# cvjena/mvlm

Hardware: NVIDIA B200
Metric: scans/sec (higher is better)
Workload: dtype bf16

## Files before the change

mvlm_b200/csrc/hourglass.cu:

```cuda
#include "hourglass.cuh"

#include <math.h>
#include <stdlib.h>

#include <algorithm>

namespace mvlm {

namespace {

__global__ void fold_bn_kernel(const float* w, const float* b, const float* m, const float* v, float eps, int n,
                               float* scale, float* shift) {
  const int i = blockIdx.x * blockDim.x + threadIdx.x;
  if (i >= n) return;
  const float s = w[i] / sqrtf(v[i] + eps);
  scale[i] = s;
  shift[i] = b[i] - m[i] * s;
}

__global__ void pack_conv_weight_kernel(const float* __restrict__ w, int cout, int cin, int kh, int kw,
                                        int cout_pad, int cin_pad, __nv_bfloat16* __restrict__ out) {
  const long long total = 1ll * cout_pad * kw * kh * cin_pad;
  for (long long i = blockIdx.x * 1ll * blockDim.x + threadIdx.x; i < total;
       i += 1ll * gridDim.x * blockDim.x) {
// ... 60 lines not shown
}

int pack_conv_weight(const float* w_oihw, int cout, int cin, int kh, int kw, int cout_pad, int cin_pad,
                     __nv_bfloat16* out, cudaStream_t stream) {
  const long long total = 1ll * cout_pad * kw * kh * cin_pad;
  const int block = 256;
  const int grid = static_cast<int>((total + block - 1) / block > 4096 ? 4096 : (total + block - 1) / block);
  pack_conv_weight_kernel<<<grid, block, 0, stream>>>(w_oihw, cout, cin, kh, kw, cout_pad, cin_pad, out);
  MVLM_CHECK_CUDA(cudaGetLastError());
  return MVLM_OK;
}

HourglassNet::~HourglassNet() {
  for (auto& g : graphs_) cudaGraphExecDestroy(g.second);
  for (void* p : owned_) cudaFree(p);
}

static uint8_t* const kFakeBase = reinterpret_cast<uint8_t*>(static_cast<uintptr_t>(1) << 44);

void* HourglassNet::ws_alloc(size_t bytes) {
  const size_t aligned = (bytes + 1023) & ~static_cast<size_t>(1023);
  if (layout_pass_) {
    Buf b;
    b.bytes = aligned;
    b.fake_off = fake_off_;
    bufs_.push_back(b);
    fake_off_ += aligned;
    return kFakeBase + b.fake_off;
  }
  if (ws_ == nullptr || next_buf_ >= bufs_.size()) return nullptr;
  return ws_ + bufs_[next_buf_++].offset;
}

void HourglassNet::note_use(const void* p) {
  if (!layout_pass_ || p == nullptr) return;
  const uint8_t* q = static_cast<const uint8_t*>(p);
  if (q < kFakeBase || q >= kFakeBase + fake_off_) return;
  const size_t off = static_cast<size_t>(q - kFakeBase);
  size_t lo = 0, hi = bufs_.size();
  while (hi - lo > 1) {
    const size_t mid = (lo + hi) / 2;
    if (bufs_[mid].fake_off <= off) lo = mid; else hi = mid;
  }
  Buf& b = bufs_[lo];
  const int op = static_cast<int>(ops_.size());
  if (b.first < 0) b.first = op;
  b.last = std::max(b.last, op);
}

void HourglassNet::note_conv(const void* in, const ConvEpilogue& e) {
  note_use(in); note_use(e.out_pre); note_use(e.res1); note_use(e.res2); note_use(e.res_up); note_use(e.out_raw);
  note_use(e.out_post); note_use(e.argmax_keys); note_use(e.out_aux1); note_use(e.out_aux2);
}

void HourglassNet::assign_offsets() {
  const int n_ops = static_cast<int>(ops_.size());
  for (Buf& b : bufs_) {
    if (b.first < 0) { b.first = 0; b.last = n_ops; }
    if (b.pinned || !reuse_) { b.first = 0; b.last = n_ops; }
  }
  std::vector<size_t> order(bufs_.size());
  for (size_t i = 0; i < order.size(); ++i) order[i] = i;
  std::stable_sort(order.begin(), order.end(), [&](size_t a, size_t b) { return bufs_[a].first < bufs_[b].first; });
  struct Block { size_t off, bytes; };
  std::vector<Block> free_list;
  std::vector<size_t> live;
  size_t top = 0;
  auto release = [&](size_t id) {
    Block nb = {bufs_[id].offset, bufs_[id].bytes};
    size_t k = 0;
    while (k < free_list.size() && free_list[k].off < nb.off) ++k;
    free_list.insert(free_list.begin() + k, nb);
    for (size_t j = 0; j + 1 < free_list.size();) {
      if (free_list[j].off + free_list[j].bytes == free_list[j + 1].off) {
        free_list[j].bytes += free_list[j + 1].bytes;
        free_list.erase(free_list.begin() + j + 1);
      } else {
        ++j;
      }
    }
    if (!free_list.empty() && free_list.back().off + free_list.back().bytes == top) {
      top = free_list.back().off;
      free_list.pop_back();
    }
  };
  for (size_t id : order) {
    Buf& b = bufs_[id];
    for (size_t j = 0; j < live.size();) {
      if (bufs_[live[j]].last < b.first) {
// ... 95 lines not shown
}

int HourglassNet::stem_weight(const __nv_bfloat16** out) {
  void* buf;
  const float* src;
  const int rc = param("conv1.weight", 64ll * cin_ * 9, sizeof(__nv_bfloat16) * 64 * 9 * 16, &buf, &src);
  *out = static_cast<__nv_bfloat16*>(buf);
  if (rc || layout_pass_) return rc;
  pack_stem_weight_kernel<<<36, 256, 0, build_stream_>>>(src, 64, cin_, 64, static_cast<__nv_bfloat16*>(buf));
  MVLM_CHECK_CUDA(cudaGetLastError());
  return MVLM_OK;
}

int HourglassNet::phase_weight(int a, int b, const __nv_bfloat16** out) {
  void* buf;
  const float* src;
  const int rc = param("conv11.weight", 9ll * L_ * L_, sizeof(__nv_bfloat16) * Lp_ * 4 * Lp_, &buf, &src);
  *out = static_cast<__nv_bfloat16*>(buf);
  if (rc || layout_pass_) return rc;
  pack_phase_weight_kernel<<<64, 256, 0, build_stream_>>>(src, L_, L_, a, b, Lp_, Lp_, static_cast<__nv_bfloat16*>(buf));
  MVLM_CHECK_CUDA(cudaGetLastError());
  return MVLM_OK;
}

int HourglassNet::emit_conv(const char* tag, T in, int cin, const __nv_bfloat16* w, int cout_pad, int n_tile, int kh,
                            int kw, int y_off0, int x_off0, const ConvEpilogue& e, double flops, bool is_head) {
  flops_ += flops;
  note_conv(in.p, e);
  NetOp op;
  op.kind = NetOp::CONV;
  op.tag = tag;
  op.is_head = is_head;
  op.h = in.h; op.w = in.w;
  if (!layout_pass_) {
    ConvShape s;
    s.in = in.p; s.n = V_; s.h = in.h; s.w = in.w; s.cin = cin; s.in_cs = in.c;
    s.wpacked = w; s.cout_pad = cout_pad; s.n_tile = n_tile; s.kh = kh; s.kw = kw;
    s.y_off0 = y_off0; s.x_off0 = x_off0;
    const int rc = conv_plan(s, e, &op.conv);
    if (rc) return rc;
  }
  ops_.push_back(op);
  return MVLM_OK;
}

int HourglassNet::rb(const std::string& p, T x, T a_in, T ar, int cin, int cout, const char* post_bn, T* post_act,
                     T* y_out, T* pool_raw, const T* up_low, const RbAux* aux) {
  const int h = a_in.h, w = a_in.w;
  T y = alloc(h, w, cout);
  T skip = x;
  int rc;
  if (cin != cout) {
    ConvEpilogue e;
    e.out_raw = y.p; e.raw_cs = cout; e.raw_co = 0;
    const __nv_bfloat16* wr;
    if ((rc = packed(p + ".resample.2.weight", cout, cin, 1, cout, cin, &wr)) ||
        (rc = emit_conv("rb.resample", ar, cin, wr, cout, cout < 128 ? cout : 128, 1, 1, 0, 0, e,
                        2.0 * cout * cin * ar.h * ar.w)))
      return rc;
    skip = y;
  }
  const float *ps = nullptr, *pt = nullptr;
  if (post_bn) {
    rc = bn(post_bn, cout, &ps, &pt);
    if (rc) return rc;
    *post_act = pool_raw ? alloc(h / 2, w / 2, cout) : alloc(h, w, cout);
  }
  if (pool_raw) *pool_raw = alloc(h / 2, w / 2, cout);
  const float *as = nullptr, *at = nullptr;
  if (aux) {
    rc = bn(aux->bn, cout, &as, &at);
    if (rc) return rc;
    *aux->out1 = aux->mode == 2 ? alloc(h / 2, w / 2, cout) : alloc(h, w, cout);
// ... 27 lines not shown
    }
    if (aux) {
      e.aux_mode = aux->mode;
      e.aux_scale = layout_pass_ ? nullptr : as + offs[i];
      e.aux_shift = layout_pass_ ? nullptr : at + offs[i];
      e.out_aux1 = aux->out1->p; e.aux1_cs = cout; e.aux1_co = offs[i];
      if (aux->mode == 2) { e.out_aux2 = aux->out2->p; e.aux2_cs = cout; e.aux2_co = offs[i]; }
    }
    const int nt = widths[i] < 128 ? widths[i] : 128;
    const __nv_bfloat16* wc;
    if ((rc = packed(p + names[i] + ".weight", widths[i], cins[i], 3, widths[i], cins[i], &wc)) ||
        (rc = emit_conv("rb.conv", ins[i], cins[i], wc, widths[i], nt, 3, 3, -1, -1, e,
                        2.0 * widths[i] * cins[i] * 9 * h * w)))
      return rc;
  }
  *y_out = y;
  return MVLM_OK;
}

int HourglassNet::emit_pool(T in, T out_raw, const char* bn_name, T out_act) {
  note_use(in.p); note_use(out_raw.p); note_use(out_act.p);
  NetOp op;
  op.kind = NetOp::POOL;
  op.in0 = in.p; op.out_raw = out_raw.p; op.out_act = out_act.p;
  op.h = in.h; op.w = in.w; op.c = in.c;
  if (bn_name) {
    int rc = bn(bn_name, in.c, &op.scale, &op.shift);
    if (rc) return rc;
  }
  ops_.push_back(op);
  return MVLM_OK;
}

int HourglassNet::hourglass(const std::string& p, T x, T a_x, T* out, const T* in_pooled, const T* in_pooled_act) {
  const int F = 256;
  int rc;
  T none;
  T lows[5], a_lows[5];
  T cur = x;
  const int low_blocks[5] = {2, 4, 6, 8, 10};
  const int skip_blocks[4] = {3, 5, 7, 9};
  T pooled, a;
  if (in_pooled) {
    pooled = *in_pooled;
    a = *in_pooled_act;
  }
  for (int lvl = 0; lvl < 5; ++lvl) {
    const std::string lb = p + ".rb" + std::to_string(low_blocks[lvl]);
    if (!(fuse_elt_ && (lvl > 0 || in_pooled))) {
      pooled = alloc(cur.h / 2, cur.w / 2, F);
      a = alloc(cur.h / 2, cur.w / 2, F);
      rc = emit_pool(cur, pooled, (lb + ".bn1").c_str(), a);
      if (rc) return rc;
    }
    const int nxt = lvl < 4 ? skip_blocks[lvl] : 11;
    const std::string post = p + ".rb" + std::to_string(nxt) + ".bn1";
    T next_pooled, next_a;
    const std::string next_bn = lvl < 4 ? p + ".rb" + std::to_string(low_blocks[lvl + 1]) + ".bn1" : "";
    RbAux aux = {2, next_bn.c_str(), &next_pooled, &next_a};
    rc = rb(lb, pooled, a, none, F, F, post.c_str(), &a_lows[lvl], &lows[lvl], nullptr, nullptr,
            (fuse_elt_ && lvl < 4) ? &aux : nullptr);
    if (rc) return rc;
    cur = lows[lvl];
    pooled = next_pooled;
    a = next_a;
  }
  T low2, a2, low3;
  rc = rb(p + ".rb11", cur, a_lows[4], none, F, F, (p + ".rb12.bn1").c_str(), &a2, &low2);
  if (rc) return rc;
  rc = rb(p + ".rb12", low2, a2, none, F, F, nullptr, nullptr, &low3);
  if (rc) return rc;
  cur = low3;
  const int ups[4][2] = {{13, 14}, {15, 16}, {17, 18}, {19, 20}};
  for (int lvl = 0; lvl < 4; ++lvl) {
    const std::string sb = p + ".rb" + std::to_string(skip_blocks[3 - lvl]);
    const std::string b1 = p + ".rb" + std::to_string(ups[lvl][0]);
    const std::string b2 = p + ".rb" + std::to_string(ups[lvl][1]);
    T s, a;
    rc = rb(sb, lows[3 - lvl], a_lows[3 - lvl], none, F, F, (b1 + ".bn1").c_str(), &a, &s, nullptr, &cur);
    if (rc) return rc;
    T l1, a1, l2;
    rc = rb(b1, s, a, none, F, F, (b2 + ".bn1").c_str(), &a1, &l1);
    if (rc) return rc;
    rc = rb(b2, l1, a1, none, F, F, nullptr, nullptr, &l2);
    if (rc) return rc;
    cur = l2;
  }
  T add5;
  rc = rb(p + ".rb1", x, a_x, none, F, F, nullptr, nullptr, &add5, nullptr, &cur);
  if (rc) return rc;
  *out = add5;
  return MVLM_OK;
}

int HourglassNet::build(const StateDict* sd, int n_landmarks, int cin, int n_views, int h,
                        int w, void* workspace, size_t workspace_bytes, bool dry) {
  MVLM_REQUIRE(n_landmarks > 0 && n_landmarks <= 128, "hourglass: n_landmarks=%d unsupported", n_landmarks);
  MVLM_REQUIRE(cin >= 1 && cin <= 4, "hourglass: image channels=%d unsupported", cin);
  MVLM_REQUIRE(n_views > 0 && h >= 64 && w >= 64 && h % 64 == 0 && w % 64 == 0,
               "hourglass: image size %dx%d must be a positive multiple of 64", h, w);
  MVLM_REQUIRE(dry || (sd && workspace), "hourglass: null state_dict/workspace");
  sd_ = sd;
  V_ = n_views; H_ = h; W_ = w; L_ = n_landmarks; cin_ = cin;
  Lp_ = pad_to(L_, 16);
  if (Lp_ == 112) Lp_ = 128;
  if (Lp_ == 48) Lp_ = 64;
  if (Lp_ == 16) Lp_ = 32;
  ws_ = static_cast<uint8_t*>(workspace); ws_size_ = workspace_bytes;
  keep_probes_ = getenv("MVLM_HG_KEEP_PROBES") != nullptr && atoi(getenv("MVLM_HG_KEEP_PROBES")) != 0;
  reuse_ = !(getenv("MVLM_HG_NO_REUSE") != nullptr && atoi(getenv("MVLM_HG_NO_REUSE")) != 0);
  fuse_elt_ = !(getenv("MVLM_HG_ELT_FUSION") != nullptr && atoi(getenv("MVLM_HG_ELT_FUSION")) == 0);
  bufs_.clear(); fake_off_ = 0; ws_needed_ = 0; next_buf_ = 0;
  layout_pass_ = true;
  int rc = emit();
  layout_pass_ = false;
  if (rc) return rc;
  assign_offsets();
  if (dry) return MVLM_OK;
  MVLM_REQUIRE(ws_needed_ <= ws_size_, "hourglass: workspace too small (%zu needed, %zu given)", ws_needed_, ws_size_);
  const size_t param_bytes = param_off_ + 4096;
  MVLM_CHECK_CUDA(cudaMalloc(&params_, param_bytes));
  owned_.push_back(params_);
  param_cap_ = param_bytes;
  MVLM_CHECK_CUDA(cudaStreamCreateWithFlags(&build_stream_, cudaStreamNonBlocking));
  rc = emit();
  if (rc == MVLM_OK && param_off_ > param_bytes) {
    set_error("hourglass: parameter arena overrun (%zu of %zu bytes)", param_off_, param_bytes);
    rc = MVLM_E_INVALID;
  }
  const cudaError_t ce = cudaStreamSynchronize(build_stream_);
  cudaStreamDestroy(build_stream_);
  build_stream_ = nullptr;
  if (rc) return rc;
  MVLM_CHECK_CUDA(ce);
  return MVLM_OK;
}

void HourglassNet::probe(const char* name, const T& t) {
  probes[name] = {t.p, t.h, t.w, t.c};
  if (layout_pass_ && keep_probes_ && t.p) {
    const size_t off = static_cast<size_t>(reinterpret_cast<const uint8_t*>(t.p) - kFakeBase);
    for (Buf& b : bufs_)
      if (b.fake_off == off) b.pinned = true;
  }
}

int HourglassNet::emit() {
  const int h = H_, w = W_, cin = cin_;
  ops_.clear(); flops_ = 0.0; probes.clear();
  param_off_ = 0; bn_cache_.clear();
  int rc;
  const int F = 256, h2 = h / 2, w2 = w / 2;

  T a_c2 = alloc(h, w, 64), ar_c2 = alloc(h, w, 64);
  T img16 = alloc(h, w, 16);
  {
    note_use(img16.p);
    NetOp op;
    op.kind = NetOp::STEM;
    op.out_raw = img16.p; op.h = h; op.w = w; op.c = cin;
    ops_.push_back(op);
    const __nv_bfloat16* w1;
    ConvEpilogue e;
    if ((rc = stem_weight(&w1))) return rc;
    if ((rc = bias("conv1.bias", 64, 64, &e.bias))) return rc;
    if ((rc = bn("bn1", 64, &e.mid_scale, &e.mid_shift))) return rc;
    if ((rc = bn("conv2.bn1", 64, &e.pre_scale, &e.pre_shift))) return rc;
    if ((rc = bn("conv2.resample.0", 64, &e.post_scale, &e.post_shift))) return rc;
    e.out_pre = a_c2.p; e.pre_cs = 64; e.pre_co = 0;
    e.out_post = ar_c2.p; e.post_cs = 64; e.post_co = 0;
    if ((rc = emit_conv("conv1", img16, 16, w1, 64, 64, 3, 3, -1, -1, e, 2.0 * 64 * cin * 9 * h * w))) return rc;
  }
  T none, y2, y3, r3, a3, a4, a_h1, ar4;
  T x1;
  if ((rc = rb("conv2", none, a_c2, ar_c2, 64, 128, "conv3.bn1", &a3, &y2, &x1))) return rc;
  probe("x1", x1);
  if (fuse_elt_) {
    RbAux aux = {1, "conv4.resample.0", &ar4, nullptr};
    if ((rc = rb("conv3", x1, a3, none, 128, 128, "conv4.bn1", &a4, &y3, nullptr, nullptr, &aux))) return rc;
    probe("y3", y3);
  } else {
    if ((rc = rb("conv3", x1, a3, none, 128, 128, "conv4.bn1", &a4, &y3))) return rc;
// ... 98 lines not shown
          (rc = emit_conv("conv11.phase", x10, Lp_, phase_w_[2 * a + b], Lp_, Lp_, 2, 2, a - 1, b - 1, e,
                          2.0 * L_ * L_ * 9 * h2 * w2, true)))
        return rc;
    }
  }
  {
    note_use(keys_);
    note_use(x10.p);
    NetOp op;
    op.kind = NetOp::PEAKS;
    ops_.push_back(op);
  }
  return MVLM_OK;
}

int HourglassNet::run_op(NetOp& op, const unsigned char* img_u8, const float* img_f32, float* out_heatmaps,
                         float* out_peaks, cudaStream_t stream) {
  unsigned long long* const keys = out_keys_ ? out_keys_ : keys_;
  switch (op.kind) {
    case NetOp::STEM:
      return image_to_hilo16(img_u8, img_f32, op.c, static_cast<size_t>(V_) * op.h * op.w, op.out_raw, stream);
    case NetOp::CONV:
      if (op.is_head) {
        ConvParams p = op.conv;
        p.e.out_f32 = out_heatmaps;
        p.e.argmax_keys = keys;
        return conv_launch(p, stream);
      }
      return conv_launch(op.conv, stream);
    case NetOp::POOL:
      return pool2_act(op.in0, V_, op.h, op.w, op.c, op.out_raw, op.scale, op.shift, op.out_act, stream);
    case NetOp::BNRELU:
      return bn_relu(op.in0, static_cast<size_t>(V_) * op.h * op.w, op.c, op.scale, op.shift, op.out_act, stream);
    case NetOp::MEMSET:
      MVLM_CHECK_CUDA(cudaMemsetAsync(keys, 0, op.bytes, stream));
      return MVLM_OK;
    case NetOp::PEAKS:
      if (out_peaks && !out_keys_) {
        if (peak_method_ == 1)
          return peaks_moment_from_keys(keys_, x10_, Lp_, Lp_, phase_w_, b11_, V_, L_, H_, W_, out_peaks, stream);
        return peaks_from_keys(keys_, V_, L_, H_, W_, out_peaks, stream);
      }
      return MVLM_OK;
  }
  return MVLM_OK;
}

int HourglassNet::set_selection_method(int method) {
  MVLM_REQUIRE(method == 0 || method == 1, "hourglass: unknown selection method %d", method);
  if (method != peak_method_) {
    for (auto& g : graphs_) cudaGraphExecDestroy(g.second);
    graphs_.clear();
    peak_method_ = method;
  }
  return MVLM_OK;
}

int HourglassNet::forward_keys(const unsigned char* img_u8, const float* img_f32, unsigned long long* out_keys,
                               cudaStream_t stream) {
  MVLM_REQUIRE(out_keys, "hourglass: null key buffer");
  out_keys_ = out_keys;
  const int rc = forward_graph(img_u8, img_f32, nullptr, reinterpret_cast<float*>(out_keys), stream);
  out_keys_ = nullptr;
  return rc;
}

// ... 11 lines not shown
int HourglassNet::profile_ops(const unsigned char* img_u8, const float* img_f32, float* out_peaks, int reps,
                              float* ms_out, double* roles_out, int trace_op, long long* trace_out,
                              cudaStream_t stream) {
  MVLM_REQUIRE(params_ && out_peaks && ms_out && reps > 0, "hourglass: bad profile_ops arguments");
  const size_t n = ops_.size();
  std::vector<cudaEvent_t> ev(n + 1);
  for (auto& e : ev) MVLM_CHECK_CUDA(cudaEventCreate(&e));
  for (size_t i = 0; i < n; ++i) ms_out[i] = 0.f;
  int rc = forward(img_u8, img_f32, nullptr, out_peaks, stream);
  for (int r = 0; r < reps && rc == MVLM_OK; ++r) {
    MVLM_CHECK_CUDA(cudaEventRecord(ev[0], stream));
    for (size_t i = 0; i < n && rc == MVLM_OK; ++i) {
      rc = run_op(ops_[i], img_u8, img_f32, nullptr, out_peaks, stream);
      MVLM_CHECK_CUDA(cudaEventRecord(ev[i + 1], stream));
    }
    MVLM_CHECK_CUDA(cudaStreamSynchronize(stream));
    for (size_t i = 0; i < n; ++i) {
      float ms = 0.f;
      MVLM_CHECK_CUDA(cudaEventElapsedTime(&ms, ev[i], ev[i + 1]));
      ms_out[i] += ms / reps;
    }
  }
  for (auto& e : ev) cudaEventDestroy(e);
  if (roles_out && rc == MVLM_OK) {
    long long* dev = nullptr;
    MVLM_CHECK_CUDA(cudaMalloc(&dev, sizeof(long long) * kConvProfInts));
    std::vector<long long> host(kConvProfInts);
    for (size_t i = 0; i < n && rc == MVLM_OK; ++i) {
      for (int k = 0; k < 8; ++k) roles_out[i * 8 + k] = 0.0;
      if (ops_[i].kind == NetOp::CONV) {
        MVLM_CHECK_CUDA(cudaMemsetAsync(dev, 0, sizeof(long long) * kConvProfInts, stream));
        conv_set_profile_buffer(dev);
      }
      rc = run_op(ops_[i], img_u8, img_f32, nullptr, out_peaks, stream);
      conv_set_profile_buffer(nullptr);
      if (ops_[i].kind == NetOp::CONV && rc == MVLM_OK) {
        MVLM_CHECK_CUDA(cudaStreamSynchronize(stream));
        MVLM_CHECK_CUDA(cudaMemcpy(host.data(), dev, sizeof(long long) * kConvProfInts, cudaMemcpyDeviceToHost));
        if (trace_out && static_cast<int>(i) == trace_op)
          for (int k = 0; k < kConvTraceTiles * 16; ++k) trace_out[k] = host[kNumSMs * 8 + k];
        int ctas = 0;
        for (int c = 0; c < kNumSMs; ++c) {
          if (host[c * 8 + 4] == 0) continue;
          ++ctas;
          for (int k = 0; k < 8; ++k) roles_out[i * 8 + k] += static_cast<double>(host[c * 8 + k]);
        }
        for (int k = 0; k < 8; ++k) roles_out[i * 8 + k] /= ctas > 0 ? ctas : 1;
      }
    }
    cudaFree(dev);
  }
  return rc;
}

std::string HourglassNet::describe_op(int i) const {
  if (i < 0 || i >= static_cast<int>(ops_.size())) return "";
  const NetOp& op = ops_[i];
  char buf[256];
  switch (op.kind) {
    case NetOp::CONV: {
      const ConvShape& s = op.conv.s;
      const ConvEpilogue& e = op.conv.e;
      snprintf(buf, sizeof(buf), "conv %s %dx%d %d->%d k%d%s%s%s%s%s%s%s%s", op.tag, s.h, s.w, s.cin, s.cout_pad, s.kh,
               e.out_pre ? " pre" : "", e.res1 ? " res1" : "", e.res2 ? " res2" : "", e.res_up ? " up" : "", e.out_raw ? " raw" : "",
               e.out_post ? " post" : "", e.pool2 ? " pool" : (e.aux_mode == 2 ? " +pooled" : (e.aux_mode == 1 ? " +act2" : "")),
               e.argmax_keys ? " argmax" : "");
      break;
    }
    case NetOp::POOL: snprintf(buf, sizeof(buf), "pool %dx%dx%d", op.h, op.w, op.c); break;
    case NetOp::BNRELU: snprintf(buf, sizeof(buf), "bnrelu %dx%dx%d", op.h, op.w, op.c); break;
    case NetOp::STEM: snprintf(buf, sizeof(buf), "stem-stage %dx%dx%d", op.h, op.w, op.c); break;
    case NetOp::MEMSET: snprintf(buf, sizeof(buf), "memset %zu", op.bytes); break;
    case NetOp::PEAKS: snprintf(buf, sizeof(buf), "peaks"); break;
  }
  return buf;
}

int HourglassNet::forward_graph(const unsigned char* img_u8, const float* img_f32, float* out_heatmaps,
                                float* out_peaks, cudaStream_t stream) {
  for (auto& g : graphs_) {
    if (g.first.a == img_u8 && g.first.b == img_f32 && g.first.c == out_heatmaps && g.first.d == out_peaks) {
      MVLM_CHECK_CUDA(cudaGraphLaunch(g.second, stream));
      count_launch(static_cast<int>(ops_.size()));
      return MVLM_OK;
    }
  }
  int rc = forward(img_u8, img_f32, out_heatmaps, out_peaks, stream);
  if (rc != MVLM_OK) return rc;
  if (graphs_.size() >= kMaxGraphs) {
    cudaGraphExecDestroy(graphs_.front().second);
    graphs_.erase(graphs_.begin());
  }
  cudaGraph_t graph = nullptr;
  if (cudaStreamBeginCapture(stream, cudaStreamCaptureModeThreadLocal) != cudaSuccess) {
    cudaGetLastError();
    return MVLM_OK;
  }
  rc = forward(img_u8, img_f32, out_heatmaps, out_peaks, stream);
  const cudaError_t ce = cudaStreamEndCapture(stream, &graph);
  if (rc != MVLM_OK || ce != cudaSuccess || !graph) {
    cudaGetLastError();
    if (graph) cudaGraphDestroy(graph);
    return rc;
  }
  cudaGraphExec_t exec = nullptr;
  if (cudaGraphInstantiate(&exec, graph, 0) == cudaSuccess && exec) {
// ... 12 lines not shown
```

mvlm_b200/csrc/hourglass.cuh:

```cuda
#pragma once
#include <map>
#include <string>
#include <vector>

#include "conv_umma.cuh"
#include "stages.cuh"

namespace mvlm {

struct SdEntry {
  const float* p = nullptr;
  long long numel = -1;
};
typedef std::map<std::string, SdEntry> StateDict;

struct NetOp {
  enum Kind { CONV, POOL, BNRELU, STEM, MEMSET, PEAKS } kind;
  ConvParams conv;
  const __nv_bfloat16* in0 = nullptr;
  __nv_bfloat16* out_raw = nullptr;
  __nv_bfloat16* out_act = nullptr;
  const float* scale = nullptr;
  const float* shift = nullptr;
  int h = 0, w = 0, c = 0;
  size_t bytes = 0;
  bool is_head = false;
  const char* tag = "";
};

class HourglassNet {
 public:
  HourglassNet() = default;
  ~HourglassNet();
  int build(const StateDict* sd, int n_landmarks, int cin, int n_views, int h, int w,
            void* workspace, size_t workspace_bytes, bool dry);
  int forward(const unsigned char* img_u8, const float* img_f32, float* out_heatmaps, float* out_peaks,
              cudaStream_t stream);
  int run_op(NetOp& op, const unsigned char* img_u8, const float* img_f32, float* out_heatmaps, float* out_peaks,
             cudaStream_t stream);
  int forward_graph(const unsigned char* img_u8, const float* img_f32, float* out_heatmaps, float* out_peaks,
                    cudaStream_t stream);

  int set_selection_method(int method);
  int forward_keys(const unsigned char* img_u8, const float* img_f32, unsigned long long* out_keys, cudaStream_t stream);

  int profile_ops(const unsigned char* img_u8, const float* img_f32, float* out_peaks, int reps, float* ms_out,
                  double* roles_out, int trace_op, long long* trace_out, cudaStream_t stream);
  std::string describe_op(int i) const;

  size_t workspace_needed() const { return ws_needed_; }
  int n_views() const { return V_; }
  int n_landmarks() const { return L_; }
  int height() const { return H_; }
  int width() const { return W_; }
  double flops_per_view() const { return flops_; }
  int n_ops() const { return static_cast<int>(ops_.size()); }
  const std::vector<NetOp>& ops() const { return ops_; }
  struct Probe { const __nv_bfloat16* p; int h, w, c; };
  std::map<std::string, Probe> probes;

 private:
  struct T { __nv_bfloat16* p = nullptr; int h = 0, w = 0, c = 0; };
  T alloc(int h, int w, int c);
  void* ws_alloc(size_t bytes);
  struct Buf {
    size_t bytes = 0, fake_off = 0, offset = 0;
    int first = -1, last = -1;
    bool pinned = false;
  };
  int emit();
  void note_use(const void* p);
  void note_conv(const void* in, const ConvEpilogue& e);
  void assign_offsets();
  void probe(const char* name, const T& t);
  int param(const std::string& name, long long numel, size_t bytes, void** dst, const float** src);
  unsigned char* params_ = nullptr;
  size_t param_off_ = 0, param_cap_ = 0;
  cudaStream_t build_stream_ = nullptr;
  static constexpr size_t kMaxGraphs = 8;
  std::vector<Buf> bufs_;
  size_t fake_off_ = 0, ws_needed_ = 0, next_buf_ = 0;
  bool layout_pass_ = false, keep_probes_ = false, reuse_ = true, fuse_elt_ = false;
  int bn(const std::string& name, int c, const float** scale, const float** shift);
  int packed(const std::string& name, int cout, int cin, int k, int cout_pad, int cin_pad, const __nv_bfloat16** out);
  int bias(const std::string& name, int cout, int cout_pad, const float** out);
  int stem_weight(const __nv_bfloat16** out);
  int phase_weight(int a, int b, const __nv_bfloat16** out);
  int emit_conv(const char* tag, T in, int cin, const __nv_bfloat16* w, int cout_pad, int n_tile, int kh, int kw,
                int y_off0, int x_off0, const ConvEpilogue& e, double flops, bool is_head = false);
  struct RbAux { int mode; const char* bn; T* out1; T* out2; };
  int rb(const std::string& p, T x, T a_in, T ar, int cin, int cout, const char* post_bn, T* post_act, T* y_out,
         T* pool_raw = nullptr, const T* up_low = nullptr, const RbAux* aux = nullptr);
  int hourglass(const std::string& p, T x, T a_x, T* out, const T* in_pooled = nullptr, const T* in_pooled_act = nullptr);
  int emit_pool(T in, T out_raw, const char* bn_name, T out_act);

  const StateDict* sd_ = nullptr;
  int sd_get(const std::string& name, long long numel, const float** out) const;
  int V_ = 0, H_ = 0, W_ = 0, L_ = 0, Lp_ = 0, cin_ = 0;
  uint8_t* ws_ = nullptr;
  size_t ws_size_ = 0;
  std::vector<void*> owned_;
  std::map<std::string, std::pair<float*, float*>> bn_cache_;
  std::vector<NetOp> ops_;
  unsigned long long* keys_ = nullptr;
  unsigned long long* out_keys_ = nullptr;
  int peak_method_ = 0;
  const __nv_bfloat16* phase_w_[4] = {nullptr, nullptr, nullptr, nullptr};
  const float* b11_ = nullptr;
  const __nv_bfloat16* x10_ = nullptr;
  double flops_ = 0.0;
  struct GraphKey { const void* a; const void* b; const void* c; const void* d; };
  std::vector<std::pair<GraphKey, cudaGraphExec_t>> graphs_;
};

}
```

Before: 62.60.

## Fuse low-resolution hourglass residual blocks into one persistent tcgen05 kernel

Captures the chain of 3x3 residual-block convolutions at the smallest hourglass levels (maps up to 8x8) and replaces them with a single persistent kernel per view. Activations stay in shared memory and weights stream through a TMA ring into UMMA with TMEM accumulators. This removes many tiny, launch- and latency-bound conv kernels and their global round trips. The cost is a complex warp-specialised kernel, stricter shape validation, and fewer CTAs (one per view), which could underuse the GPU.

```diff
diff --git a/mvlm_b200/csrc/hourglass.cu b/mvlm_b200/csrc/hourglass.cu
--- a/mvlm_b200/csrc/hourglass.cu
+++ b/mvlm_b200/csrc/hourglass.cu
@@ -116,7 +116,7 @@
   return ws_ + bufs_[next_buf_++].offset;
 }
 
-void HourglassNet::note_use(const void* p) {
+void HourglassNet::note_use_at(const void* p, const int op) {
   if (!layout_pass_ || p == nullptr) return;
   const uint8_t* q = static_cast<const uint8_t*>(p);
   if (q < kFakeBase || q >= kFakeBase + fake_off_) return;
@@ -127,8 +127,7 @@
     if (bufs_[mid].fake_off <= off) lo = mid; else hi = mid;
   }
   Buf& b = bufs_[lo];
-  const int op = static_cast<int>(ops_.size());
-  if (b.first < 0) b.first = op;
+  b.first = b.first < 0 ? op : std::min(b.first, op);
   b.last = std::max(b.last, op);
 }
 
@@ -138,7 +137,7 @@
 }
 
 void HourglassNet::assign_offsets() {
-  const int n_ops = static_cast<int>(ops_.size());
+  const int n_ops = op_index();
   for (Buf& b : bufs_) {
     if (b.first < 0) { b.first = 0; b.last = n_ops; }
     if (b.pinned || !reuse_) { b.first = 0; b.last = n_ops; }
@@ -300,13 +299,21 @@
   op.tag = tag;
   op.is_head = is_head;
   op.h = in.h; op.w = in.w;
+  ConvShape s;
+  s.in = in.p; s.n = V_; s.h = in.h; s.w = in.w; s.cin = cin; s.in_cs = in.c;
+  s.wpacked = w; s.cout_pad = cout_pad; s.n_tile = n_tile; s.kh = kh; s.kw = kw;
+  s.y_off0 = y_off0; s.x_off0 = x_off0;
   if (!layout_pass_) {
-    ConvShape s;
-    s.in = in.p; s.n = V_; s.h = in.h; s.w = in.w; s.cin = cin; s.in_cs = in.c;
-    s.wpacked = w; s.cout_pad = cout_pad; s.n_tile = n_tile; s.kh = kh; s.kw = kw;
-    s.y_off0 = y_off0; s.x_off0 = x_off0;
     const int rc = conv_plan(s, e, &op.conv);
     if (rc) return rc;
+  } else {
+    op.conv.s = s;
+    op.conv.e = e;
+  }
+  if (capturing_) {
+    lowres_convs_.push_back(op.conv);
+    ++lowres_extra_;
+    return MVLM_OK;
   }
   ops_.push_back(op);
   return MVLM_OK;
@@ -400,6 +407,58 @@
   return MVLM_OK;
 }
 
+static bool lowres_map(int h, int w) { return (h <= 4 || h == 8) && w <= 8; }
+
+void HourglassNet::begin_lowres() {
+  capturing_ = true;
+  lowres_first_ = op_index();
+  lowres_convs_.clear();
+}
+
+void* HourglassNet::arena(size_t bytes) {
+  const size_t aligned = (bytes + 255) & ~static_cast<size_t>(255);
+  void* dst = (layout_pass_ || params_ == nullptr || param_off_ + aligned > param_cap_) ? nullptr : params_ + param_off_;
+  param_off_ += aligned;
+  return dst;
+}
+
+int HourglassNet::end_lowres() {
+  capturing_ = false;
+  const int n_convs = static_cast<int>(lowres_convs_.size());
+  const int n_blocks = n_convs / 3;
+  std::vector<LowresBlock> blocks(n_blocks);
+  int rc = lowres_describe(lowres_convs_.data(), n_convs, blocks.data());
+  if (rc) return rc;
+  const int first = lowres_first_, last = op_index() - 1;
+  for (int b = 0; b < n_blocks; ++b) {
+    if (!blocks[b].load) continue;
+    for (const void* q : {static_cast<const void*>(lowres_convs_[3 * b].s.in), static_cast<const void*>(blocks[b].x)}) {
+      note_use_at(q, first);
+      note_use_at(q, last);
+    }
+  }
+  __nv_bfloat16* const out = lowres_convs_.back().e.out_raw;
+  note_use_at(out, first); note_use_at(out, last);
+  NetOp op;
+  op.kind = NetOp::LOWRES;
+  op.tag = "lowres";
+  op.h = blocks.back().h; op.w = blocks.back().w;
+  op.lowres.n_blocks = n_blocks;
+  op.lowres.n_views = V_;
+  op.lowres.out = out;
+  void* dst = arena(sizeof(LowresBlock) * n_blocks);
+  op.lowres.blocks = static_cast<const LowresBlock*>(dst);
+  if (!layout_pass_) {
+    MVLM_REQUIRE(dst, "hourglass: parameter arena exhausted (LOWRES blocks)");
+    lowres_host_.push_back(std::move(blocks));
+    MVLM_CHECK_CUDA(cudaMemcpyAsync(dst, lowres_host_.back().data(), sizeof(LowresBlock) * n_blocks,
+                                    cudaMemcpyHostToDevice, build_stream_));
+  }
+  ops_.push_back(op);
+  --lowres_extra_;
+  return MVLM_OK;
+}
+
 int HourglassNet::hourglass(const std::string& p, T x, T a_x, T* out, const T* in_pooled, const T* in_pooled_act) {
   const int F = 256;
   int rc;
@@ -421,6 +480,7 @@
       rc = emit_pool(cur, pooled, (lb + ".bn1").c_str(), a);
       if (rc) return rc;
     }
+    if (lvl == 4 && lowres_ && lowres_map(pooled.h, pooled.w)) begin_lowres();
     const int nxt = lvl < 4 ? skip_blocks[lvl] : 11;
     const std::string post = p + ".rb" + std::to_string(nxt) + ".bn1";
     T next_pooled, next_a;
@@ -441,6 +501,7 @@
   cur = low3;
   const int ups[4][2] = {{13, 14}, {15, 16}, {17, 18}, {19, 20}};
   for (int lvl = 0; lvl < 4; ++lvl) {
+    if (capturing_ && (lvl > 0 || !lowres_map(lows[3 - lvl].h, lows[3 - lvl].w)) && (rc = end_lowres())) return rc;
     const std::string sb = p + ".rb" + std::to_string(skip_blocks[3 - lvl]);
     const std::string b1 = p + ".rb" + std::to_string(ups[lvl][0]);
     const std::string b2 = p + ".rb" + std::to_string(ups[lvl][1]);
@@ -454,6 +515,7 @@
     if (rc) return rc;
     cur = l2;
   }
+  if (capturing_ && (rc = end_lowres())) return rc;
   T add5;
   rc = rb(p + ".rb1", x, a_x, none, F, F, nullptr, nullptr, &add5, nullptr, &cur);
   if (rc) return rc;
@@ -478,6 +540,7 @@
   keep_probes_ = getenv("MVLM_HG_KEEP_PROBES") != nullptr && atoi(getenv("MVLM_HG_KEEP_PROBES")) != 0;
   reuse_ = !(getenv("MVLM_HG_NO_REUSE") != nullptr && atoi(getenv("MVLM_HG_NO_REUSE")) != 0);
   fuse_elt_ = !(getenv("MVLM_HG_ELT_FUSION") != nullptr && atoi(getenv("MVLM_HG_ELT_FUSION")) == 0);
+  lowres_ = !(getenv("MVLM_HG_LOWRES") != nullptr && atoi(getenv("MVLM_HG_LOWRES")) == 0);
   bufs_.clear(); fake_off_ = 0; ws_needed_ = 0; next_buf_ = 0;
   layout_pass_ = true;
   int rc = emit();
@@ -516,6 +579,7 @@
 int HourglassNet::emit() {
   const int h = H_, w = W_, cin = cin_;
   ops_.clear(); flops_ = 0.0; probes.clear();
+  capturing_ = false; lowres_extra_ = 0; lowres_convs_.clear(); lowres_host_.clear();
   param_off_ = 0; bn_cache_.clear();
   int rc;
   const int F = 256, h2 = h / 2, w2 = w / 2;
@@ -680,6 +744,8 @@
       return pool2_act(op.in0, V_, op.h, op.w, op.c, op.out_raw, op.scale, op.shift, op.out_act, stream);
     case NetOp::BNRELU:
       return bn_relu(op.in0, static_cast<size_t>(V_) * op.h * op.w, op.c, op.scale, op.shift, op.out_act, stream);
+    case NetOp::LOWRES:
+      return lowres_launch(op.lowres, stream);
     case NetOp::MEMSET:
       MVLM_CHECK_CUDA(cudaMemsetAsync(keys, 0, op.bytes, stream));
       return MVLM_OK;
@@ -757,8 +823,18 @@
         MVLM_CHECK_CUDA(cudaMemsetAsync(dev, 0, sizeof(long long) * kConvProfInts, stream));
         conv_set_profile_buffer(dev);
       }
+      const bool lowres_trace = ops_[i].kind == NetOp::LOWRES && trace_out && static_cast<int>(i) == trace_op;
+      if (lowres_trace) {
+        MVLM_CHECK_CUDA(cudaMemsetAsync(dev, 0, sizeof(long long) * kLowresTraceInts, stream));
+        lowres_set_trace_buffer(dev);
+      }
       rc = run_op(ops_[i], img_u8, img_f32, nullptr, out_peaks, stream);
       conv_set_profile_buffer(nullptr);
+      lowres_set_trace_buffer(nullptr);
+      if (lowres_trace && rc == MVLM_OK) {
+        MVLM_CHECK_CUDA(cudaStreamSynchronize(stream));
+        MVLM_CHECK_CUDA(cudaMemcpy(trace_out, dev, sizeof(long long) * kLowresTraceInts, cudaMemcpyDeviceToHost));
+      }
       if (ops_[i].kind == NetOp::CONV && rc == MVLM_OK) {
         MVLM_CHECK_CUDA(cudaStreamSynchronize(stream));
         MVLM_CHECK_CUDA(cudaMemcpy(host.data(), dev, sizeof(long long) * kConvProfInts, cudaMemcpyDeviceToHost));
@@ -797,6 +873,9 @@
     case NetOp::STEM: snprintf(buf, sizeof(buf), "stem-stage %dx%dx%d", op.h, op.w, op.c); break;
     case NetOp::MEMSET: snprintf(buf, sizeof(buf), "memset %zu", op.bytes); break;
     case NetOp::PEAKS: snprintf(buf, sizeof(buf), "peaks"); break;
+    case NetOp::LOWRES:
+      snprintf(buf, sizeof(buf), "lowres %d blocks up to %dx%d", op.lowres.n_blocks, op.h, op.w);
+      break;
   }
   return buf;
 }
diff --git a/mvlm_b200/csrc/hourglass.cuh b/mvlm_b200/csrc/hourglass.cuh
--- a/mvlm_b200/csrc/hourglass.cuh
+++ b/mvlm_b200/csrc/hourglass.cuh
@@ -4,6 +4,7 @@
 #include <vector>
 
 #include "conv_umma.cuh"
+#include "lowres.cuh"
 #include "stages.cuh"
 
 namespace mvlm {
@@ -15,8 +16,9 @@
 typedef std::map<std::string, SdEntry> StateDict;
 
 struct NetOp {
-  enum Kind { CONV, POOL, BNRELU, STEM, MEMSET, PEAKS } kind;
+  enum Kind { CONV, POOL, BNRELU, STEM, MEMSET, PEAKS, LOWRES } kind;
   ConvParams conv;
+  LowresParams lowres;
   const __nv_bfloat16* in0 = nullptr;
   __nv_bfloat16* out_raw = nullptr;
   __nv_bfloat16* out_act = nullptr;
@@ -69,7 +71,9 @@
     bool pinned = false;
   };
   int emit();
-  void note_use(const void* p);
+  void note_use(const void* p) { note_use_at(p, op_index()); }
+  void note_use_at(const void* p, int op);
+  int op_index() const { return static_cast<int>(ops_.size()) + lowres_extra_; }
   void note_conv(const void* in, const ConvEpilogue& e);
   void assign_offsets();
   void probe(const char* name, const T& t);
@@ -80,7 +84,12 @@
   static constexpr size_t kMaxGraphs = 8;
   std::vector<Buf> bufs_;
   size_t fake_off_ = 0, ws_needed_ = 0, next_buf_ = 0;
-  bool layout_pass_ = false, keep_probes_ = false, reuse_ = true, fuse_elt_ = false;
+  bool layout_pass_ = false, keep_probes_ = false, reuse_ = true, fuse_elt_ = false, lowres_ = false;
+  bool capturing_ = false;
+  int lowres_extra_ = 0;
+  int lowres_first_ = 0;
+  std::vector<ConvParams> lowres_convs_;
+  std::vector<std::vector<LowresBlock>> lowres_host_;
   int bn(const std::string& name, int c, const float** scale, const float** shift);
   int packed(const std::string& name, int cout, int cin, int k, int cout_pad, int cin_pad, const __nv_bfloat16** out);
   int bias(const std::string& name, int cout, int cout_pad, const float** out);
@@ -93,6 +102,9 @@
          T* pool_raw = nullptr, const T* up_low = nullptr, const RbAux* aux = nullptr);
   int hourglass(const std::string& p, T x, T a_x, T* out, const T* in_pooled = nullptr, const T* in_pooled_act = nullptr);
   int emit_pool(T in, T out_raw, const char* bn_name, T out_act);
+  void begin_lowres();
+  int end_lowres();
+  void* arena(size_t bytes);
 
   const StateDict* sd_ = nullptr;
   int sd_get(const std::string& name, long long numel, const float** out) const;
diff --git a/mvlm_b200/csrc/lowres.cu b/mvlm_b200/csrc/lowres.cu
--- /dev/null
+++ b/mvlm_b200/csrc/lowres.cu
@@ -0,0 +1,407 @@
+#include "conv_epilogue.cuh"
+#include "lowres.cuh"
+
+#include <atomic>
+
+namespace mvlm {
+
+namespace {
+
+using namespace epi;
+
+constexpr int kLrThreads = 320;
+constexpr int kLrEpiWarps = 8;
+constexpr int kFrameW = 10;
+constexpr int kChunkBytes = 13 * 1024;
+constexpr int kSlotBytes = 16 * 1024;
+constexpr int kSlots = 4;
+constexpr int kRawBytes = 64 * 256 * 2;
+constexpr int kLowBytes = 16 * 256 * 2;
+constexpr int kStageBytes = kLrEpiWarps * kStageFloats * 4;
+constexpr int kOffA = 0;
+constexpr int kOffA1 = kOffA + 4 * kChunkBytes;
+constexpr int kOffA2 = kOffA1 + 2 * kChunkBytes;
+constexpr int kOffRing = kOffA2 + kChunkBytes;
+constexpr int kOffRaw = kOffRing + kSlots * kSlotBytes;
+constexpr int kOffLow = kOffRaw + kRawBytes;
+constexpr int kOffStage = kOffLow + kLowBytes;
+constexpr int kOffBar = kOffStage + kStageBytes;
+constexpr int kLrSmemBytes = kOffBar + 512 + 1024 ;
+static_assert(kFrameW * kFrameW * 128 <= kChunkBytes, "frame chunk");
+static_assert(kOffRing % 1024 == 0 && kOffA1 % 1024 == 0 && kOffA2 % 1024 == 0, "swizzle atoms");
+static_assert(kLrSmemBytes <= 227 * 1024, "shared memory budget");
+
+struct __align__(8) LrBarriers {
+  uint64_t w_full[kSlots];
+  uint64_t w_empty[kSlots];
+  uint64_t t_full;
+  uint64_t act_ready;
+  uint64_t in_full;
+  uint32_t tmem_base;
+};
+static_assert(sizeof(LrBarriers) <= 512, "barrier block");
+
+__device__ __forceinline__ void epi_sync() { asm volatile("bar.sync 1, %0;" ::"n"(kLrEpiWarps * 32) : "memory"); }
+
+__device__ __forceinline__ uint4* frame_at(uint8_t* frame, int y, int x, int c) {
+  const int row = (y + 1) * kFrameW + (x + 1);
+  return reinterpret_cast<uint4*>(frame + (c >> 6) * kChunkBytes + row * 128 + ((((c & 63) >> 3) ^ (row & 7)) << 4));
+}
+
+__device__ __forceinline__ void ldg8(const float* p, float (&v)[8]) {
+  const float4 a = __ldg(reinterpret_cast<const float4*>(p));
+  const float4 b = __ldg(reinterpret_cast<const float4*>(p) + 1);
+  v[0] = a.x; v[1] = a.y; v[2] = a.z; v[3] = a.w; v[4] = b.x; v[5] = b.y; v[6] = b.z; v[7] = b.w;
+}
+
+__device__ __forceinline__ int tile_rows(int i, int h) { return (i > 0 || h >= 8) ? 8 : 4; }
+
+__global__ void __launch_bounds__(kLrThreads, 1) lowres_kernel(const __grid_constant__ LowresParams p) {
+  extern __shared__ uint8_t smem_raw[];
+  const uint32_t raw_addr = ptx::smem_u32(smem_raw);
+  uint8_t* smem = smem_raw + ((1024u - (raw_addr & 1023u)) & 1023u);
+  uint8_t* const fA = smem + kOffA;
+  uint8_t* const fA1 = smem + kOffA1;
+  uint8_t* const fA2 = smem + kOffA2;
+  uint8_t* const ring = smem + kOffRing;
+  uint4* const raw = reinterpret_cast<uint4*>(smem + kOffRaw);
+  uint4* const low = reinterpret_cast<uint4*>(smem + kOffLow);
+  LrBarriers* bar = reinterpret_cast<LrBarriers*>(smem + kOffBar);
+  const int warp = threadIdx.x >> 5;
+  const int lane = threadIdx.x & 31;
+  const int n_blocks = p.n_blocks;
+
+  if (warp == 0 && lane == 0) {
+    for (int i = 0; i < kSlots; ++i) {
+      ptx::mbar_init(&bar->w_full[i], 1);
+      ptx::mbar_init(&bar->w_empty[i], 1);
+    }
+    ptx::mbar_init(&bar->t_full, 1);
+    ptx::mbar_init(&bar->act_ready, kLrEpiWarps);
+    ptx::mbar_init(&bar->in_full, 1);
+    ptx::fence_mbar_init();
+  }
+  if (warp == 0) {
+    ptx::tmem_alloc(&bar->tmem_base, 128);
+    ptx::tmem_relinquish();
+  }
+  ptx::tc_fence_before();
+  __syncthreads();
+  ptx::tc_fence_after();
+  const uint32_t tmem_base = bar->tmem_base;
+  long long* const trace = blockIdx.x == 0 ? p.prof : nullptr;
+  const long long t0 = clock64();
+
+  if (warp == 1) {
+    if (ptx::elect_one()) {
+      int sw = 0;
+      uint32_t pw = 0;
+      for (int view = blockIdx.x; view < p.n_views; view += gridDim.x) {
+        for (int b = 0; b < n_blocks; ++b) {
+          const LowresBlock* blk = p.blocks + b;
+          for (int i = 0; i < 3; ++i) {
+            const int cin = 256 >> i;
+            const uint32_t bytes = (i == 0 ? 128u : 64u) * 128u;
+            for (int c = 0; c < cin / 64; ++c) {
+              for (int tap = 0; tap < 9; ++tap) {
+                ptx::mbar_wait_trap(&bar->w_empty[sw], pw ^ 1);
+                ptx::mbar_expect_tx(&bar->w_full[sw], bytes);
+                ptx::tma_load_2d(&blk->tm_w[i], &bar->w_full[sw], ring + sw * kSlotBytes, tap * cin + c * 64, 0);
+                if (++sw == kSlots) { sw = 0; pw ^= 1; }
+              }
+            }
+          }
+        }
+      }
+    }
+  } else {
+    asm volatile("griddepcontrol.wait;" ::: "memory");
+    asm volatile("griddepcontrol.launch_dependents;" ::: "memory");
+    if (warp == 0) {
+      if (ptx::elect_one()) {
+        const uint64_t a_hi = static_cast<uint64_t>(((8u * 128u) >> 4) | (1u << 14) | (2u << 29)) << 32;
+        const uint64_t b_hi = static_cast<uint64_t>(((kFrameW * 128u) >> 4) | (1u << 14) | (2u << 29)) << 32;
+        const uint32_t ring_lo = (ptx::smem_u32(ring) >> 4) | (1u << 16);
+        const uint32_t frame_lo[3] = {(ptx::smem_u32(fA) >> 4) | (1u << 16), (ptx::smem_u32(fA1) >> 4) | (1u << 16),
+                                      (ptx::smem_u32(fA2) >> 4) | (1u << 16)};
+        int sw = 0;
+        uint32_t pw = 0, pa = 0, pin = 0;
+        int lay = 0;
+        for (int view = blockIdx.x; view < p.n_views; view += gridDim.x) {
+          for (int b = 0; b < n_blocks; ++b) {
+            const LowresBlock* blk = p.blocks + b;
+            const int h = blk->h;
+            const bool load = blk->load != 0;
+            for (int i = 0; i < 3; ++i, ++lay) {
+              ptx::mbar_wait_trap(&bar->act_ready, pa);
+              pa ^= 1;
+              if (i == 0 && load) {
+                ptx::mbar_wait_trap(&bar->in_full, pin);
+                pin ^= 1;
+              }
+              ptx::tc_fence_after();
+              if (trace && lay < kLowresTraceLayers) trace[lay * 4 + 0] = clock64() - t0;
+              const uint32_t idesc = i == 0 ? ptx::umma_idesc_bf16(kMTile, 8 * tile_rows(0, h)) : ptx::umma_idesc_bf16(64, 64);
+              const int n_chunks = 4 >> i;
+              uint32_t accumulate = 0;
+              for (int c = 0; c < n_chunks; ++c) {
+                const uint32_t x_chunk = frame_lo[i] + static_cast<uint32_t>(c * (kChunkBytes >> 4));
+                for (int kx = 0; kx < 3; ++kx) {
+                  for (int ky = 0; ky < 3; ++ky) {
+                    ptx::mbar_wait_trap(&bar->w_full[sw], pw);
+                    const uint32_t x_lo = x_chunk + static_cast<uint32_t>((ky * kFrameW + kx) * 8);
+                    const uint32_t w_lo = ring_lo + static_cast<uint32_t>(sw * (kSlotBytes >> 4));
+#pragma unroll
+                    for (int k = 0; k < 4; ++k) {
+                      if (i == 0) ptx::umma_bf16(tmem_base, a_hi | (w_lo + 2 * k), b_hi | (x_lo + 2 * k), idesc, k == 0 ? accumulate : 1u);
+                      else ptx::umma_ws_bf16(tmem_base, a_hi | (w_lo + 2 * k), b_hi | (x_lo + 2 * k), idesc, k == 0 ? accumulate : 1u);
+                    }
+                    accumulate = 1;
+                    ptx::umma_commit(&bar->w_empty[sw]);
+                    if (++sw == kSlots) { sw = 0; pw ^= 1; }
+                  }
+                }
+              }
+              ptx::umma_commit(&bar->t_full);
+              if (trace && lay < kLowresTraceLayers) trace[lay * 4 + 1] = clock64() - t0;
+            }
+          }
+        }
+      }
+    } else {
+      const int ew = warp - 2;
+      const int lane_grp = warp & 3;
+      const int half = ew >> 2;
+      const int tid = threadIdx.x - 64;
+      float* const stage = reinterpret_cast<float*>(smem + kOffStage) + ew * kStageFloats;
+      constexpr int kPitch = 36;
+      const int pj = lane >> 2;
+      const int cq = (lane & 3) * 8;
+      uint32_t pt = 0;
+      int lay = 0;
+      auto arrive = [&]() {
+        ptx::fence_proxy_async();
+        ptx::tc_fence_before();
+        __syncwarp();
+        if (lane == 0) ptx::mbar_arrive(&bar->act_ready);
+      };
+      uint4 xpre[8];
+      auto fetch_level = [&](const LowresBlock* nb, int nview) {
+        const int n = nb->h * nb->w * 32;
+        if (tid == 0) {
+          const uint32_t bytes = 64u * 2u * kFrameW * static_cast<uint32_t>(tile_rows(0, nb->h) + 2);
+          ptx::mbar_expect_tx(&bar->in_full, 4u * bytes);
+          for (int c = 0; c < 4; ++c) ptx::tma_load_4d(&nb->tm_a, &bar->in_full, fA + c * kChunkBytes, c * 64, -1, -1, nview);
+        }
+        const uint4* xg = reinterpret_cast<const uint4*>(nb->x) + static_cast<size_t>(nview) * n;
+#pragma unroll
+        for (int q = 0; q < 8; ++q)
+          if (tid + q * kLrEpiWarps * 32 < n) xpre[q] = xg[tid + q * kLrEpiWarps * 32];
+      };
+      if (static_cast<int>(blockIdx.x) < p.n_views) fetch_level(p.blocks, blockIdx.x);
+      for (int view = blockIdx.x; view < p.n_views; view += gridDim.x) {
+        for (int k = tid; k < 3 * kChunkBytes / 16; k += kLrEpiWarps * 32)
+          reinterpret_cast<uint4*>(fA1)[k] = make_uint4(0u, 0u, 0u, 0u);
+        for (int b = 0; b < n_blocks; ++b) {
+          const LowresBlock* blk = p.blocks + b;
+          const int h = blk->h, w = blk->w;
+          if (blk->load) {
+            epi_sync();
+            if (blk->up) {
+              const int hl = h >> 1, wl = w >> 1;
+              for (int k = tid; k < hl * wl * 32; k += kLrEpiWarps * 32) {
+                const int px = k >> 5, j = k & 31, yy = px / wl, xx = px % wl;
+                low[(yy * 4 + xx) * 32 + j] = raw[(yy * 8 + xx) * 32 + j];
+              }
+              epi_sync();
+            }
+#pragma unroll
+            for (int q = 0; q < 8; ++q) {
+              const int k = tid + q * kLrEpiWarps * 32;
+              if (k < h * w * 32) raw[(((k >> 5) / w) * 8 + (k >> 5) % w) * 32 + (k & 31)] = xpre[q];
+            }
+            epi_sync();
+            arrive();
+          }
+          const bool up = blk->up != 0;
+          const LowresBlock* next_load = nullptr;
+          int next_view = view;
+          if (b + 1 < n_blocks) {
+            if (p.blocks[b + 1].load) next_load = p.blocks + b + 1;
+          } else if (view + static_cast<int>(gridDim.x) < p.n_views) {
+            next_load = p.blocks;
+            next_view = view + gridDim.x;
+          }
+          for (int i = 0; i < 3; ++i, ++lay) {
+            const bool ws = i > 0;
+            const int n_cols = 8 * tile_rows(i, h);
+            const int cbase = ws ? (lane_grp & 1) * 32 : lane_grp * 32;
+            const int n_units = ws ? 2 : n_cols / 16;
+            const int upw = n_units / 2;
+            const int pix0 = ws ? (lane_grp >> 1) * 32 : 0;
+            const int off = i == 0 ? 0 : (i == 1 ? 128 : 192);
+            const bool pre = i < 2;
+            const bool post = blk->post_s != nullptr;
+            float pre_s[8], pre_t[8], post_s[8], post_t[8];
+            const int c0 = cbase + cq;
+            if (pre) { ldg8(blk->pre_s[i] + c0, pre_s); ldg8(blk->pre_t[i] + c0, pre_t); }
+            if (post) { ldg8(blk->post_s + off + c0, post_s); ldg8(blk->post_t + off + c0, post_t); }
+            uint8_t* const f_pre = i == 0 ? fA1 : fA2;
+            ptx::mbar_wait_trap(&bar->t_full, pt);
+            pt ^= 1;
+            ptx::tc_fence_after();
+            if (trace && ew == 0 && lane == 0 && lay < kLowresTraceLayers) trace[lay * 4 + 2] = clock64() - t0;
+            if (i == 0 && next_load) fetch_level(next_load, next_view);
+            float fr[2][2][8];
+            bool ok[2][2];
+#pragma unroll
+            for (int r = 0; r < 2; ++r) {
+              const int col = (half * upw + r) * 16;
+              const int pb = pix0 + col;
+              ok[r][0] = ok[r][1] = false;
+              if (r >= upw || (pb >> 3) >= h) continue;
+              uint32_t vr[16];
+              ptx::tmem_ld16(tmem_base + (static_cast<uint32_t>(lane_grp * 32) << 16) + static_cast<uint32_t>(col), vr);
+              ptx::tmem_ld_wait();
+              __syncwarp();
+#pragma unroll
+              for (int j = 0; j < 16; ++j) stage[j * kPitch + lane] = __uint_as_float(vr[j]) + 0.f;
+              __syncwarp();
+#pragma unroll
+              for (int ip = 0; ip < 2; ++ip) {
+                const int y = (pb >> 3) + ip, x = pj;
+                ok[r][ip] = y < h && x < w;
+                if (ok[r][ip]) {
+                  lds8(stage + (pj + 8 * ip) * kPitch + cq, fr[r][ip]);
+                  if (pre) *frame_at(f_pre, y, x, c0) = affine_relu_pack8(fr[r][ip], pre_s, pre_t);
+                }
+              }
+            }
+            if (pre) arrive();
+#pragma unroll
+            for (int r = 0; r < 2; ++r) {
+              const int pb = pix0 + (half * upw + r) * 16;
+#pragma unroll
+              for (int ip = 0; ip < 2; ++ip) {
+                if (!ok[r][ip]) continue;
+                const int y = (pb >> 3) + ip, x = pj;
+                uint4* const rp = raw + (y * 8 + x) * 32 + ((off + c0) >> 3);
+                add8(*rp, fr[r][ip]);
+                if (up) add8(low[((y >> 1) * 4 + (x >> 1)) * 32 + ((off + c0) >> 3)], fr[r][ip]);
+                *rp = pack8(fr[r][ip]);
+                if (post) *frame_at(fA, y, x, off + c0) = affine_relu_pack8(fr[r][ip], post_s, post_t);
+              }
+            }
+            if (trace && ew == 0 && lane == 0 && lay < kLowresTraceLayers) trace[lay * 4 + 3] = clock64() - t0;
+            if (!pre && b + 1 < n_blocks && !p.blocks[b + 1].load) arrive();
+          }
+        }
+        epi_sync();
+        const int h = p.blocks[n_blocks - 1].h, w = p.blocks[n_blocks - 1].w;
+        uint4* const og = reinterpret_cast<uint4*>(p.out) + static_cast<size_t>(view) * h * w * 32;
+        for (int k = tid; k < h * w * 32; k += kLrEpiWarps * 32) {
+          const int px = k >> 5, j = k & 31;
+          og[k] = raw[((px / w) * 8 + px % w) * 32 + j];
+        }
+      }
+    }
+  }
+  ptx::tc_fence_before();
+  __syncthreads();
+  if (warp == 0) {
+    ptx::tc_fence_after();
+    ptx::tmem_dealloc(tmem_base, 128);
+  }
+}
+
+thread_local long long* g_trace_buf = nullptr;
+
+}
+
+void lowres_set_trace_buffer(long long* dev_buf) { g_trace_buf = dev_buf; }
+
+int lowres_describe(const ConvParams* convs, int n_convs, LowresBlock* blocks) {
+  MVLM_REQUIRE(n_convs > 0 && n_convs % 3 == 0, "lowres: %d convolutions do not form ResidualBlocks", n_convs);
+  const int n_blocks = n_convs / 3;
+  const __nv_bfloat16* prev_y = nullptr;
+  const __nv_bfloat16* prev_post = nullptr;
+  for (int b = 0; b < n_blocks; ++b) {
+    const ConvParams* c = convs + 3 * b;
+    LowresBlock& blk = blocks[b];
+    blk = LowresBlock();
+    const int h = c[0].s.h, w = c[0].s.w;
+    for (int i = 0; i < 3; ++i) {
+      const ConvShape& s = c[i].s;
+      const ConvEpilogue& e = c[i].e;
+      MVLM_REQUIRE(s.cin == (256 >> i) && s.cout_pad == (i == 0 ? 128 : 64) && s.kh == 3 && s.kw == 3 && s.y_off0 == -1 &&
+                       s.x_off0 == -1 && s.h == h && s.w == w && (h <= 4 || h == 8) && w <= 8,
+                   "lowres: block %d conv %d is not a 3x3 %d -> %d convolution of a map the kernel holds", b, i, 256 >> i,
+                   i == 0 ? 128 : 64);
+      MVLM_REQUIRE(!e.bias && !e.mid_scale && !e.res2 && !e.pool2 && e.aux_mode == 0 && !e.out_f32 && !e.argmax_keys &&
+                       e.res1 && e.out_raw && e.res1_cs == 256 && e.raw_cs == 256 && e.res1_co == (i == 0 ? 0 : 64 + 64 * i) &&
+                       e.raw_co == e.res1_co && (!e.res_up || (e.up_cs == 256 && e.up_co == e.res1_co)) &&
+                       (!e.out_post || (e.post_cs == 256 && e.post_co == e.res1_co)) &&
+                       (i == 2 ? !e.out_pre : (e.out_pre != nullptr && e.pre_cs == (128 >> i) && e.pre_co == 0)),
+                   "lowres: block %d conv %d has an epilogue the kernel does not implement", b, i);
+      MVLM_REQUIRE(e.res1 == c[0].e.res1 && e.out_raw == c[0].e.out_raw && e.res_up == c[0].e.res_up &&
+                       e.out_post == c[0].e.out_post && (i == 0 || s.in == c[i - 1].e.out_pre),
+                   "lowres: block %d conv %d does not continue the block", b, i);
+    }
+    MVLM_REQUIRE(!c[0].e.out_post || !c[0].e.post_scale ||
+                     (c[1].e.post_scale == c[0].e.post_scale + 128 && c[2].e.post_scale == c[0].e.post_scale + 192 &&
+                      c[1].e.post_shift == c[0].e.post_shift + 128 && c[2].e.post_shift == c[0].e.post_shift + 192),
+                 "lowres: block %d: post BatchNorm slices", b);
+    blk.h = h;
+    blk.w = w;
+    blk.up = c[0].e.res_up != nullptr;
+    blk.load = b == 0 || c[0].e.res1 != prev_y;
+    MVLM_REQUIRE(!blk.up || (blk.load && c[0].e.res_up == prev_y && h == 2 * blocks[b - 1].h && w == 2 * blocks[b - 1].w),
+                 "lowres: block %d adds an up-sampled tensor that is not the previous block's output", b);
+    MVLM_REQUIRE(blk.load == (b == 0 || blk.up), "lowres: block %d starts a level that is not an up level", b);
+    MVLM_REQUIRE(blk.load || c[0].s.in == prev_post, "lowres: block %d does not read the previous block's activation", b);
+    MVLM_REQUIRE(!blk.load || (c[0].s.in_cs == 256 && c[0].e.res1_co == 0), "lowres: block %d input strides", b);
+    MVLM_REQUIRE(!c[0].e.out_post || (b + 1 < n_blocks && convs[3 * (b + 1)].s.in == c[0].e.out_post),
+                 "lowres: block %d writes an activation no block of the op reads", b);
+    if (blk.load) {
+      blk.x = c[0].e.res1;
+      blk.tm_a = c[0].tm_a;
+    }
+    for (int i = 0; i < 3; ++i) blk.tm_w[i] = c[i].tm_b;
+    blk.pre_s[0] = c[0].e.pre_scale; blk.pre_t[0] = c[0].e.pre_shift;
+    blk.pre_s[1] = c[1].e.pre_scale; blk.pre_t[1] = c[1].e.pre_shift;
+    blk.post_s = c[0].e.out_post ? c[0].e.post_scale : nullptr;
+    blk.post_t = c[0].e.out_post ? c[0].e.post_shift : nullptr;
+    prev_y = c[0].e.out_raw;
+    prev_post = c[0].e.out_post;
+  }
+  return MVLM_OK;
+}
+
+int lowres_launch(const LowresParams& p_in, cudaStream_t stream) {
+  LowresParams p = p_in;
+  p.prof = g_trace_buf;
+  static std::atomic<bool> configured[kMaxDevices];
+  int dev = 0;
+  MVLM_CHECK_CUDA(cudaGetDevice(&dev));
+  if (dev < 0 || dev >= kMaxDevices || !configured[dev].load(std::memory_order_acquire)) {
+    MVLM_CHECK_CUDA(cudaFuncSetAttribute(lowres_kernel, cudaFuncAttributeMaxDynamicSharedMemorySize, kLrSmemBytes));
+    if (dev >= 0 && dev < kMaxDevices) configured[dev].store(true, std::memory_order_release);
+  }
+  const int n_sms = sm_count();
+  cudaLaunchConfig_t cfg = {};
+  cfg.gridDim = dim3(static_cast<unsigned>(p.n_views < n_sms ? p.n_views : n_sms));
+  cfg.blockDim = dim3(kLrThreads);
+  cfg.dynamicSmemBytes = kLrSmemBytes;
+  cfg.stream = stream;
+  cudaLaunchAttribute attr[1];
+  attr[0].id = cudaLaunchAttributeProgrammaticStreamSerialization;
+  attr[0].val.programmaticStreamSerializationAllowed = 1;
+  cfg.attrs = attr;
+  cfg.numAttrs = 1;
+  MVLM_CHECK_CUDA(cudaLaunchKernelEx(&cfg, lowres_kernel, p));
+  count_launch();
+  MVLM_CHECK_CUDA(cudaGetLastError());
+  return MVLM_OK;
+}
+
+}
diff --git a/mvlm_b200/csrc/lowres.cuh b/mvlm_b200/csrc/lowres.cuh
--- /dev/null
+++ b/mvlm_b200/csrc/lowres.cuh
@@ -0,0 +1,33 @@
+#pragma once
+#include "conv_umma.cuh"
+
+namespace mvlm {
+
+struct alignas(64) LowresBlock {
+  CUtensorMap tm_w[3];
+  CUtensorMap tm_a;
+  const __nv_bfloat16* x = nullptr;
+  const float* pre_s[2] = {nullptr, nullptr};
+  const float* pre_t[2] = {nullptr, nullptr};
+  const float* post_s = nullptr;
+  const float* post_t = nullptr;
+  int h = 0, w = 0;
+  int load = 0;
+  int up = 0;
+};
+
+struct LowresParams {
+  const LowresBlock* blocks = nullptr;
+  int n_blocks = 0;
+  int n_views = 0;
+  __nv_bfloat16* out = nullptr;
+  long long* prof = nullptr;
+};
+
+int lowres_describe(const ConvParams* convs, int n_convs, LowresBlock* blocks);
+int lowres_launch(const LowresParams& p, cudaStream_t stream);
+constexpr int kLowresTraceLayers = 64;
+constexpr int kLowresTraceInts = kLowresTraceLayers * 4;
+void lowres_set_trace_buffer(long long* dev_buf);
+
+}
```

Measured after the change: 63.19 (median of 6 runs). No clear change (+0.9%).
